# ebiggers/libdeflate

Measured on AMD Instinct MI355X. Metric: compress+decompress MB/s, 64 KiB chunks level 6, higher is better.
Workload: dtype u8

## Files before the change

### libdeflate_amd/csrc/deflate_kernel.hip

```cpp
#include <stddef.h>
#include "device_common.h"
#include "kernels.h"


#ifndef NT
#define NT LDA_DEFLATE_THREADS
#endif
#define VPT (1024 / NT)
#define NWAVES (NT / 64)
#ifndef TILE
#define TILE 4096
#endif
#ifndef RING
#define RING 32768u
#endif
#define RMASK (RING - 1)
#define LOOKAHEAD 272u
#ifndef HASH_BITS
#define HASH_BITS 13
#endif
#ifndef HASH3_BITS
#define HASH3_BITS 12
#endif
#define MAX_BLOCK_LEN 65536u
// ... 507 lines not shown
		const u32 w[4] = { v.x, v.y, v.z, v.w };
#pragma unroll
		for (u32 i = 0; i < 16; i++)
			if (off + i < lim)
				L->seen8[(w[i >> 2] >> (8 * (i & 3))) & 0xFF] = 1;
	}
	wave_sync();
	return wave_sum((u32)__builtin_popcount(s32p[lane] & 0x01010101u));
}

static __device__ __forceinline__ void
stage_input(lds_t *L, const u8 *__restrict__ inp, u32 loaded, u32 want,
	    bool aligned_in, u32 tid)
{
	if (aligned_in) {
		const u32 from = loaded & ~15u;
		for (u32 p = from + tid * 16; p < want; p += NT * 16) {
			uint4 v = *(const uint4 *)(inp + p);
			*(uint4 *)&L->in[p & RMASK] = v;
			if ((p & RMASK) < 32)
				*(uint4 *)&L->in[RING + (p & RMASK)] = v;
		}
	} else {
		for (u32 p = loaded + tid; p < want; p += NT) {
			u8 b = inp[p];
			L->in[p & RMASK] = b;
			if ((p & RMASK) < 32)
				L->in[RING + (p & RMASK)] = b;
		}
	}
}

static __device__ __attribute__((noinline)) void
stage_prefix(lds_t *L, const u8 *__restrict__ pre, u32 n, u32 tid)
{
	stage_input(L, pre, 0, n, true, tid);
}


struct ra_first {
	u32 c16, a0, a1, a2, a3, c3v;
};

static __device__ __forceinline__ struct ra_first
ra_first_loads(const u16 *__restrict__ c3, u32 t, u32 g, u32 lane, bool want3)
{
	struct ra_first f;
	const u32 i = 64 * g + lane, p = t + i;
	const u32 ip = (p & RMASK) & ~3u;

	f.c16 = LDS32(PREV_OFF + ((2 * (p & RMASK)) & ~3u));
	f.a0 = RAW(ip, 0);
	f.a1 = RAW(ip, 4);
	f.a2 = RAW(ip, 8);
	f.a3 = RAW(ip, 12);
	(void)want3;
	f.c3v = *(const u32 *)((const u8 *)c3 + ((2 * (4 + (g < TILE / 64 ? i : lane))) & ~3u));
	return f;
}

template <bool PRE> static __device__ __forceinline__ void
ra_group(lds_t *L, AS3 u32 *Mo, const u16 *__restrict__ c3, u32 t, u32 tend, u32 n,
	 u32 lo_pos, u32 min_len, u32 done_class, u32 nice, u32 dlim3,
	 u32 tag, u32 lane, u32 &g, const struct ra_first &f, struct ra_first &fnext)
{
	const u32 ctr = (u32)offsetof(struct deflate_lds, vars) + 4 * V_CTR;
	const bool want3 = min_len <= 3;
	const u32 i = 64 * g + lane, p = t + i;
	const u32 sp = p & 3;
	const u32 cur = AB(f.a1, f.a0, sp);
	const u64 nxt8 = mk64(AB(f.a2, f.a1, sp), AB(f.a3, f.a2, sp));
	const u32 hsh = 16 * (lane & 1);
	const u32 c3v = want3 ? (f.c3v >> hsh) & 0xFFFF : 0;
	const bool act0 = p < tend && p + 4 <= n;
	const u32 maxlen = n - p < 258 ? n - p : 258;
	const u32 dmaxp = p - lo_pos;
	const u32 nic = nice < maxlen ? nice : maxlen;
	u32 best = 3, bestd = 0;

	const u32 d1 = (p - (f.c16 >> hsh)) & 0xFFFF;
	const bool act1 = act0 && d1 > 0 && d1 <= dmaxp && 3 < nic;
	const u32 cp1 = p - d1;
	const u32 c2 = LDS16(PREV_OFF + 2 * (cp1 & RMASK));
	u32 rn = 0, gn = 0;
	if (PRE)
		rn = claim_issue(ctr);
	const u32 d2 = (p - c2) & 0xFFFF;
	const bool ch2 = act1 && d2 > d1 && d2 <= dmaxp;
	const u32 cp2 = p - d2;
	if (PRE)
		gn = claim_get(rn);
	const u32 c3n = LDS16(PREV_OFF + 2 * (cp2 & RMASK));
	u32 len1, len2;
	match_length2_p(L, act1, ch2, p, cp1, cp2, cur, nxt8, maxlen, lane,
			&len1, &len2, [&]() {
		if (PRE)
			fnext = ra_first_loads(c3, t, gn, lane, want3);
	});
	if (len1 > best) {
		best = len1;
		bestd = d1;
	}
	const bool act2 = ch2 && best < nic;
	if (act2 && len2 > best) {
		best = len2;
		bestd = d2;
	}
	u32 m = best >= 4 && best >= min_len ? best | (bestd << 16) : 0;
	if (m == 0 && want3 && p < tend && p + 3 <= n) {
		u32 b3 = 0;
		u32 bd = find_len3(L, p, cur, c3v, dmaxp, dlim3, &b3);
		if (bd)
			m = 3 | (bd << 16);
	}
	Mo[4 + i] = m;
	const u32 dn = (p - c3n) & 0xFFFF;
	const u32 dcl = act2 && dn > d2 && dn <= dmaxp && best < nic ?
			done_class : DC_FULL;
	L->dhalf[g] = __ballot(dcl >= DC_HALF);
	L->dfull[g] = __ballot(dcl == DC_FULL);
	__builtin_amdgcn_fence(__ATOMIC_RELEASE, "workgroup");
	*(volatile AS3 u32 *)&L->rdy[g] = tag;
	if (PRE) {
		g = gn;
	} else {
		g = claim_get(claim_issue(ctr));
		if (g < TILE / 64)
			fnext = ra_first_loads(c3, t, g, lane, want3);
	}
}

static __device__ __forceinline__ void
round_a_p(lds_t *L, AS3 u32 *Mo, const u16 *__restrict__ c3, u32 t, u32 tend, u32 n,
	  u32 lo_pos, u32 min_len, u32 done_class, u32 nice, u32 dlim3,
	  u32 tag, u32 tid)
{
	const u32 lane = tid & 63;
	const u32 ctr = (u32)offsetof(struct deflate_lds, vars) + 4 * V_CTR;
	u32 g = claim_get(claim_issue(ctr));
	struct ra_first f = { 0, 0, 0, 0, 0, 0 };

	if (g < TILE / 64)
		f = ra_first_loads(c3, t, g, lane, min_len <= 3);
	struct ra_first f2 = { 0, 0, 0, 0, 0, 0 };
#pragma unroll 1
	while (g + RA_PREF_TAIL < TILE / 64) {
		ra_group<true>(L, Mo, c3, t, tend, n, lo_pos, min_len, done_class, nice, dlim3,
			       tag, lane, g, f, f2);
		if (!(g + RA_PREF_TAIL < TILE / 64)) {
			f = f2;
			break;
		}
		ra_group<true>(L, Mo, c3, t, tend, n, lo_pos, min_len, done_class, nice, dlim3,
			       tag, lane, g, f2, f);
	}
#pragma unroll 1
	while (g < TILE / 64)
		ra_group<false>(L, Mo, c3, t, tend, n, lo_pos, min_len, done_class, nice, dlim3,
				tag, lane, g, f, f);
}

static __device__ __forceinline__ void
round_a(lds_t *L, AS3 u32 *Mo, const u16 *__restrict__ c3, u32 t, u32 tend, u32 n,
	u32 lo_pos, u32 min_len, u32 ra_depth, u32 done_class, u32 nice, u32 dlim3,
	u32 tag, u32 tid)
{
	const u32 lane = tid & 63;
	if (ra_depth == 2 && RA_PAIR) {
		round_a_p(L, Mo, c3, t, tend, n, lo_pos, min_len, done_class, nice, dlim3,
			  tag, tid);
		return;
	}

#pragma unroll 1
	for (;;) {
		u32 g = 0;
		if (lane == 0)
			g = atomicAdd((u32 *)&L->vars[V_CTR], 1u);
		g = bcast_first(g);
		if (g >= TILE / 64)
			break;
		const u32 i = 64 * g + lane, p = t + i;
		const u32 c3v = min_len <= 3 ? c3[4 + i] : 0;
		bool act = p < tend && p + 4 <= n;
		const u32 cur = ld32(L->in, p);
		const u64 nxt8 = ld64(L->in, p + 4);
		const u32 maxlen = n - p < 258 ? n - p : 258;
		const u32 dmaxp = p - lo_pos;
		const u32 nic = nice < maxlen ? nice : maxlen;
		u32 c16 = LDS16(PREV_OFF + 2 * (p & RMASK));
		u32 best = 3, bestd = 0, dprev = 0;

		for (u32 s = 0; s < ra_depth; s++) {
			u32 d = (p - c16) & 0xFFFF;
			act = act && d > dprev && d <= dmaxp && best < nic;
			if (!__ballot(act))
				break;
			u32 cp = p - d;
			u32 len = match_length(L, act, p, cp, cur, nxt8, maxlen, lane);
			if (len > best) {
				best = len;
				bestd = d;
			}
			if (act) {
				c16 = LDS16(PREV_OFF + 2 * (cp & RMASK));
				dprev = d;
			}
		}
		u32 m = best >= 4 && best >= min_len ? best | (bestd << 16) : 0;
		if (m == 0 && min_len <= 3 && p < tend && p + 3 <= n) {
			u32 b3 = 0;
			u32 bd = find_len3(L, p, cur, c3v, dmaxp, dlim3, &b3);
			if (bd)
				m = 3 | (bd << 16);
		}
		Mo[4 + i] = m;
		const u32 dn = (p - c16) & 0xFFFF;
		const u32 dcl = act && dn > dprev && dn <= dmaxp && best < nic ?
				done_class : DC_FULL;
		L->dhalf[g] = __ballot(dcl >= DC_HALF);
		L->dfull[g] = __ballot(dcl == DC_FULL);
		__builtin_amdgcn_fence(__ATOMIC_RELEASE, "workgroup");
		*(volatile AS3 u32 *)&L->rdy[g] = tag;
	}
}

static __device__ __forceinline__ void
stage_steps(lds_t *L, s32 limit, u32 mode, u32 nice, u32 tid)
{
	const u32 lane = tid & 63, wave = tid >> 6;

#pragma unroll
	for (u32 k = 0; k < TILE / NT; k++) {
		const u32 g = wave * (TILE / NT) + k, q = 64 * g + lane, idx = q + 4;
		u32 st = 1;
		if ((s32)q < limit)
			st = token_step(L->M[idx], L->M[idx + 1], L->M[idx + 2], mode, nice);
		const u64 b1 = __ballot(st == 1), b2 = __ballot(st == 2);
		if (lane == 0) {
			L->lit1[g] = b1;
			L->lit2[g] = b2;
		}
	}
}

static __device__ __forceinline__ void
stage_steps_claimed(lds_t *L, const AS3 u32 *Ms, s32 limit, u32 mode, u32 nice, u32 tag,
		    u32 lane)
{
	bool had = false;

#pragma unroll 1
	for (;;) {
		if (had)
			lds_add_lane0(VAR_ADDR(V_STDONE), 1u);
		const u32 g = claim_get(claim_issue(VAR_ADDR(V_CTR3)));
		if (g >= TILE / 64)
			break;
		had = true;
		while (*(volatile AS3 u32 *)&L->rdy[g] != tag ||
		       (g + 1 < TILE / 64 && *(volatile AS3 u32 *)&L->rdy[g + 1] != tag))
			__builtin_amdgcn_s_sleep(2);
		__builtin_amdgcn_fence(__ATOMIC_ACQUIRE, "workgroup");
		const u32 q = 64 * g + lane, idx = q + 4;
		u32 st = 1;
		if ((s32)q < limit)
			st = token_step(Ms[idx], Ms[idx + 1], Ms[idx + 2], mode, nice);
		L->lit1A[g] = __ballot(st == 1);
		L->lit2A[g] = __ballot(st == 2);
		__builtin_amdgcn_fence(__ATOMIC_RELEASE, "workgroup");
	}
}

static __device__ __forceinline__ void
stage_steps_cur_claimed(lds_t *L, s32 limit, u32 mode, u32 nice, u32 lane)
{
	bool had = false;

#pragma unroll 1
	for (;;) {
		if (had)
			lds_add_lane0(VAR_ADDR(V_ST2DONE), 1u);
		const u32 g = claim_get(claim_issue(VAR_ADDR(V_CTR4)));
		if (g >= TILE / 64)
			break;
		had = true;
		const u32 q = 64 * g + lane, idx = q + 4;
		u32 st = 1;
		if ((s32)q < limit)
			st = token_step(L->M[idx], L->M[idx + 1], L->M[idx + 2], mode, nice);
		L->lit1[g] = __ballot(st == 1);
		L->lit2[g] = __ballot(st == 2);
		__builtin_amdgcn_fence(__ATOMIC_RELEASE, "workgroup");
	}
}

static __device__ __forceinline__ void wait_lds_eq(lds_t *L, u32 idx, u32 val)
{
	while (*(volatile AS3 u32 *)&L->vars[idx] != val)
		__builtin_amdgcn_s_sleep(2);
	__builtin_amdgcn_fence(__ATOMIC_ACQUIRE, "workgroup");
}

static __device__ __forceinline__ s32
parse_tile(const AS3 u32 *Ms, const AS3 u64 *lit1p, const AS3 u64 *lit2p, AS3 u64 *pmp,
	   u32 lane, s32 entry, s32 limit, u64 *mask_out, u32 max_pass = 0xFFFFFFFFu)
{
	const s32 seg_lo = 64 * (s32)lane;
	const s32 hi = seg_lo + 64 < limit ? seg_lo + 64 : limit;
	const u64 lit = lane < TILE / 64 ? lit1p[lane] : 0;
	const u64 two = lane < TILE / 64 ? lit2p[lane] : 0;
	s32 ein = lane == 0 ? entry : seg_lo;
	s32 q = ein, ex = ein;
	u64 mask = 0, nm = 0;
	bool walking = q < hi;

	{
		const u64 nlit = ~lit;
		const s32 hirel = hi - seg_lo;
		const AS3 u16 *const ml = (const AS3 u16 *)(Ms + 4 + seg_lo);
		u64 starts = 0, ends = 0;
		s32 rel = q - seg_lo;
		while (__ballot(rel < hirel)) {
			if (rel < hirel) {
				const u64 x = nlit >> (u32)rel;
				const u32 left = (u32)(hirel - rel);
				u32 run = (u32)__builtin_ctzll(x | (1ull << 63));
				run = x ? run : 64;
				run = run < left ? run : left;
				const u32 r2 = (u32)rel + run;
				const bool tok = run < left;
				const u32 last = tok ? r2 : r2 - 1;
				starts |= 1ull << (u32)rel;
				ends |= 1ull << last;
				const u32 len = ml[2 * r2];
				const u32 st = (u32)(two >> (r2 & 63)) & 1 ? 2 : len;
				rel = (s32)(tok ? r2 + st : r2);
			}
		}
		if (q < hi) {
			mask = 2 * ends - starts;
			ex = seg_lo + rel;
		}
		walking = false;
	}
	for (;;) {
		while (__ballot(walking)) {
			if (walking) {
				const u32 rel = (u32)(q - seg_lo);
				const u64 inv = ~(lit >> rel);
				u32 run = inv ? (u32)__builtin_ctzll(inv) : 64;
				if (run > (u32)(hi - q))
					run = (u32)(hi - q);
				u64 add = run >= 64 ? ~0ull : (((1ull << run) - 1) << rel);
				q += (s32)run;
				if (q < hi) {
					const u32 r2 = (u32)(q - seg_lo);
					add |= 1ull << r2;
					q += (two >> r2) & 1 ? 2 : (s32)(Ms[4 + q] & 0xFFFF);
				}
				const u64 hit = add & mask;
				if (hit) {
					const u64 below = (hit & (0 - hit)) - 1;
					mask = nm | (add & below) | (mask & ~below);
					walking = false;
				} else {
					nm |= add;
					if (q >= hi) {
						mask = nm;
						ex = q;
						walking = false;
					}
				}
			}
		}
		s32 pe = (s32)__builtin_amdgcn_update_dpp((u32)ex, (u32)ex, 0x138, 0xF, 0xF, false);
		const s32 e = lane == 0 ? entry : pe;
		const bool redo = e != ein && seg_lo < limit;
		if (!__ballot(redo) || --max_pass == 0)
			break;
		nm = 0;
		if (redo) {
			ein = e;
			if (e >= hi) {
				mask = 0;
				ex = e;
			} else {
				q = e;
				walking = true;
			}
		}
	}
	if (lane < TILE / 64)
		pmp[lane] = mask;
	*mask_out = mask;
	return (s32)bcast_lane((u32)ex, limit > 0 ? (u32)(limit - 1) >> 6 : 0);
}

static __device__ __forceinline__ u32
entry_skip(const AS3 u32 *Ms, s32 entry, u32 lim_idx, u32 mode, u32 nice)
{
	u32 e = (u32)(entry + 4);

	for (u32 pre = 0; pre < 2; pre++)
		if (e < 4 && e < lim_idx)
			e += token_step(Ms[e], Ms[e + 1], Ms[e + 2], mode, nice);
	return e;
}

static __device__ __forceinline__ void
parse_and_base(lds_t *L, u32 *__restrict__ tokg, u32 t, s32 limit, u32 mode,
	       u32 nice, u32 lane)
{
	const s32 entry = (s32)bcast_first(L->vars[V_ENTRY]);
	const u32 lim_idx = (u32)(limit + 4);
	const u32 seq0 = bcast_first(L->vars[V_NSEQ]);
	u32 e = (u32)(entry + 4), npre = 0;

	for (u32 pre = 0; pre < 2; pre++) {
		if (e < 4 && e < lim_idx) {
			const u32 mm = L->M[e];
			const u32 st = token_step(mm, L->M[e + 1], L->M[e + 2], mode, nice);
			const u32 l0 = mm & 0xFFFF;
			const bool ism = st == l0 && l0;
			const u32 pos = (u32)((s32)t + (s32)e - 4);
			if (lane == 0) {
				if (ism) {
					u32 sl, xb, xv;
					tokg[seq0 + npre] = TOK_MATCH | (l0 - 3) |
							    (((mm >> 16) - 1) << 8);
					length_code(l0, &sl, &xb, &xv);
					atomicAdd((u32 *)&L->freq[257 + sl], 1u);
					dist_code(mm >> 16, &sl, &xb, &xv);
					atomicAdd((u32 *)&L->freq[288 + sl], 1u);
				} else {
					const u32 b0 = L->in[pos & RMASK];
					tokg[seq0 + npre] = b0;
					atomicAdd((u32 *)&L->freq[b0], 1u);
					if (st == 2) {
						const u32 b1 = L->in[(pos + 1) & RMASK];
						tokg[seq0 + npre + 1] = b1;
						atomicAdd((u32 *)&L->freq[b1], 1u);
					}
				}
			}
			npre += !ism && st == 2 ? 2 : 1;
			e += st;
		}
	}
	u64 mask;
	const s32 px = parse_tile((const AS3 u32 *)L->M, (const AS3 u64 *)L->lit1,
				  (const AS3 u64 *)L->lit2, (AS3 u64 *)L->pm, lane,
				  (s32)e - 4, limit, &mask);
	const u64 two = lane < TILE / 64 ? mask & L->lit2[lane] : 0;
	const u32 cnt = (u32)__builtin_popcountll(mask) + (u32)__builtin_popcountll(two);
	const u32 incl = wave_scan_incl(cnt);
	if (lane < TILE / 64)
		L->gbase[lane] = seq0 + npre + incl - cnt;
	if (lane == 63) {
		L->vars[V_NSEQ] = seq0 + npre + incl;
		L->vars[V_WALKPOS_LO] = (u32)((s32)t + px);
		L->vars[V_ENTRY] = (u32)(px - (s32)TILE);
	}
}

static __device__ __forceinline__ void
emit_groups(lds_t *L, u32 *__restrict__ tokg, u32 t, u32 lane)
{
	const u64 lt = (1ull << lane) - 1;
	bool had = false;

#pragma unroll 1
	for (;;) {
		u32 g = 0;
		asm volatile("s_waitcnt lgkmcnt(0)" ::: "memory");
		if (had)
			lds_add_lane0(VAR_ADDR(V_EMDONE), 1u);
		g = claim_get(claim_issue(VAR_ADDR(V_CTR2)));
		if (g >= TILE / 64)
			break;
		had = true;
		const u64 pmk = L->pm[g];
		if (!pmk)
			continue;
		const u64 two = pmk & L->lit2[g];
		if ((pmk >> lane) & 1) {
			const u32 q = 64 * g + lane, idx = q + 4;
			const u32 m0 = L->M[idx];
			const u32 l0 = m0 & 0xFFFF, dist = m0 >> 16;
			const u32 st = (L->lit1[g] >> lane) & 1 ? 1 : (two >> lane) & 1 ? 2 : l0;
			const u32 o = (t + q) & RMASK;
			const u32 b0 = L->in[o], b1 = L->in[o + 1];
			const u32 lsl = L->lslot[(l0 - 3) & 255];
			const u32 at = L->gbase[g] + (u32)__builtin_popcountll(pmk & lt) +
				       (u32)__builtin_popcountll(two & lt);
			const bool ism = st == l0 && l0;
			u32 dsl, xb, xv;
			dist_code(dist, &dsl, &xb, &xv);
			tokg[at] = ism ? TOK_MATCH | (l0 - 3) | ((dist - 1) << 8) : b0;
			atomicAdd((u32 *)&L->freq[ism ? 257 + lsl : b0], 1u);
			if (ism || st == 2)
				atomicAdd((u32 *)&L->freq[ism ? 288 + dsl : b1], 1u);
			if (!ism && st == 2)
				tokg[at + 1] = b1;
		}
	}
	__builtin_amdgcn_fence(__ATOMIC_RELEASE, "workgroup");
}

static __device__ __forceinline__ u32
build_worklist(lds_t *L, AS3 u32 *W, const AS3 u32 *src, u32 mode, u32 nice, u32 limit, u32 tid)
{
	const u32 lane = tid & 63, wave = tid >> 6;
	const AS3 u32 *Ms = src ? src : (const AS3 u32 *)L->M;

	u64 spill = 0;
	if (mode >= 1 && S3_HALF && wave) {
		const u32 g0 = wave * (TILE / NT), q1 = 64 * g0 - 1;
		const u64 pmask = L->pmA[g0 - 1];
		const u32 l1 = Ms[4 + q1] & 0xFFFF, l2 = Ms[4 + q1 - 1] & 0xFFFF;
		if ((pmask >> 63) && l1 >= 3 && l1 < nice)
			spill = mode >= 2 ? 3 : 1;
		if (mode >= 2 && ((pmask >> 62) & 1) && l2 >= 3 && l2 < nice)
			spill |= 1;
	}
	static_assert(S3_ROUNDS <= 1, "build_worklist() does not record the classes it hands out");
	u32 item[TILE / NT];
	u64 bal[TILE / NT];
	u64 tm_[TILE / NT], dh_[TILE / NT], df_[TILE / NT];
	u32 l0_[TILE / NT];
	u32 cw = 0;
#pragma unroll
	for (u32 k = 0; k < TILE / NT; k++) {
		const u32 g = wave * (TILE / NT) + k, q = 64 * g + lane;
		tm_[k] = L->pmA[g];
		dh_[k] = L->dhalf[g];
		df_[k] = L->dfull[g];
		const u32 mq = Ms[4 + q];
		if (src)
			L->M[4 + q] = mq;
		l0_[k] = mq & 0xFFFF;
	}
#pragma unroll
	for (u32 k = 0; k < TILE / NT; k++) {
		const u32 g = wave * (TILE / NT) + k, q = 64 * g + lane;
		const u64 tmask = bcast64(tm_[k]);
		const bool below = l0_[k] < nice;
		const u64 b = mode >= 1 && S3_HALF ?
			__ballot(lane_bit(tmask) && l0_[k] >= 3 && below) : 0;
		const u64 hmask = (b << 1) | (mode >= 2 ? b << 2 : 0) | spill;
		spill = (b >> 63) | (mode >= 2 ? b >> 62 : 0);
		const u64 wantf = tmask & ~bcast64(df_[k]);
		const u64 wanth = hmask & ~tmask & ~bcast64(dh_[k]);
		const bool isf = lane_bit(wantf);
		bal[k] = __ballot((isf || lane_bit(wanth)) && below);
		item[k] = q | ((isf ? DC_FULL : DC_HALF) << 12);
		cw += (u32)__builtin_popcountll(bal[k]);
	}
	if (lane == 0)
		L->scan[0][wave] = cw;
	__syncthreads();
	const u32 cnt_w = lane < NWAVES ? L->scan[0][lane] : 0;
	const u32 incl_w = wave_scan_incl(cnt_w);
	u32 base = bcast_lane(incl_w - cnt_w, wave);
	const u32 wc = bcast_lane(incl_w, NWAVES - 1);
#pragma unroll
	for (u32 k = 0; k < TILE / NT; k++) {
		const u32 j = base + rank_below(bal[k]);
		if (lane_bit(bal[k]) && j < limit)
			W[j] = item[k];
		base += (u32)__builtin_popcountll(bal[k]);
	}
	if (tid == 0)
		L->qn[0] = 0;
	__syncthreads();
	return bcast_first(wc < limit ? wc : limit);
}

static __device__ __forceinline__ void
search_items(lds_t *L, AS3 u32 *Mo, u32 t, u32 n, u32 lo_pos, u32 min_len, u32 depth,
	     u32 nice, const u16 *W, u32 cnt_items, u32 nwaves, u32 tid)
{
	const u32 lane = tid & 63;
	if ((tid >> 6) >= nwaves)
		return;
	const u32 drain = depth < 8 ? depth : depth >> 3 > 8 ? depth >> 3 : 8;
	const u32 half = depth >> S3_HALF_SHIFT ? depth >> S3_HALF_SHIFT : 1;
	u32 my_i = 0xFFFFFFFFu, p = 0, cur = 0, c16 = 0, dmaxp = 0,
	    maxlen = 0, dep = 0, best = 3, bestd = 0, dprev = 0,
	    cnt = 0, boff = 0, curb = 0, best0 = 3;
	u64 nxt8 = 0, q = 0;
	bool have = false, fin = true, ended = false;
	PROF_SEC_DECL;

	for (;;) {
		PROF_SEC(3);
		u64 mh = __ballot(have);
		u32 nf = __builtin_popcountll(__ballot(fin));
		if (!mh && !nf)
			break;
		if (nf && (nf >= S3_CLAIM || !mh)) {
			const u64 fm = __ballot(fin);
			u32 cbase = 0;
			if (lane == 0)
				cbase = atomicAdd((u32 *)&L->vars[V_CTR], nf);
			cbase = bcast_first(cbase);
			if (fin) {
				if (my_i < TILE && (!W || best > best0))
					Mo[4 + my_i] = best >= 4 && best >= min_len ?
						(best | (bestd << 16)) : 0;
				fin = false;
				my_i = 0xFFFFFFFFu;
				u32 it = cbase + __builtin_popcountll(fm & ((1ull << lane) - 1));
				if (it < cnt_items) {
					u32 item = W ? W[it] : it;
					my_i = item & 0xFFF;
					p = t + my_i;
					if (p + 4 <= n) {
						cur = ld32(L->in, p);
						nxt8 = ld64(L->in, p + 4);
						c16 = LDS16(PREV_OFF + 2 * (p & RMASK));
						maxlen = n - p < 258 ? n - p : 258;
						dmaxp = p - lo_pos;
						best = 3;
						bestd = 0;
						if (W) {
							dep = (item >> 12) == DC_FULL ? depth : half;
							u32 m = Mo[4 + my_i], l0 = m & 0xFFFF;
							if (l0 >= 4) {
								best = l0;
								bestd = m >> 16;
							}
						} else {
							dep = my_i >= TILE - S3_TAIL ? drain : depth;
						}
						best0 = best;
						boff = best - 3;
						curb = boff ? ld32(L->in, p + boff) : cur;
						dprev = 0;
						cnt = 0;
						ended = false;
						have = true;
						if (best >= maxlen) {
							have = false;
							fin = true;
						}
					} else {
						fin = true;
						best = best0 = 3;
					}
				}
			}
			PROF_SEC(0);
			continue;
		}
#pragma unroll
		for (int s = 0; s < S3_WALK; s++) {
			u32 d = (p - c16) & 0xFFFF;
			bool chain = dep && d > dprev && d <= dmaxp;
			bool stall = ended || cnt >= 4;
			bool ok = !stall && chain;
			u32 cp = p - d;
			u32 w = ld32(L->in, cp + boff);
			u32 c16n = LDS16(PREV_OFF + 2 * (cp & RMASK));
			bool hit = ok && w == curb;
			c16 = ok ? c16n : c16;
			dprev = ok ? d : dprev;
			dep -= ok ? 1 : 0;
			ended = ended || (!stall && !chain);
			q = hit ? ((q << 16) | d) : q;
			cnt += hit ? 1 : 0;
		}
		if (!have)
			cnt = 0;
		PROF_SEC(1);
		bool done = false;
		u32 nev = __builtin_popcountll(__ballot(cnt > 0));
		u32 nwalk = __builtin_popcountll(__ballot(have && !ended && cnt < 4));
		while (nev && (nev >= S3_EVMIN || !nwalk)) {
			bool ev = cnt > 0;
			u32 d = (u32)(q >> (16 * ((cnt - 1) & 3))) & 0xFFFF;
			cnt -= ev ? 1 : 0;
			u32 len = match_length(L, ev, p, p - d, cur, nxt8, maxlen, lane);
			if (ev && len > best) {
				best = len;
				bestd = d;
				if (len >= nice || len >= maxlen) {
					done = true;
					cnt = 0;
				} else {
					boff = len - 3;
					curb = ld32(L->in, p + boff);
				}
			}
			if (have && (done || (ended && cnt == 0))) {
				have = false;
				fin = true;
				done = false;
			}
// ... 369 lines not shown
		const bool ra_all = depth <= 4;
		const bool optm = OPT && mode == 3;
		const u32 rounds = optm || ra_all ? 0 : S3_ROUNDS;
		const u32 dlim3 = mode ? 8192u : 4096u;
		const u32 ra_depth = ra_all ? depth : S3_RA_DEPTH;
		const u32 ra_class = ra_all ? DC_FULL :
				     ra_depth >= (depth >> S3_HALF_SHIFT) ? DC_HALF : DC_SHALLOW;
		const u32 wq_limit = mode == 1 && depth < 100 && WQ_LIMIT > 64 * NWAVES ?
				     64 * NWAVES : WQ_LIMIT;
		const bool use3 = level >= 2;
		const bool splits = use3 && n - dict_len >= 5000;
		bool mx_pending = false;
		u32 tail_n = 0, tail_gen = 0, tail_e = 0;
		u32 ml_cur = 3, ml_nxt = 3;
		u32 carryv = 0;

		for (u32 it = 0; it <= num_tiles && !overflow; it++) {
			const bool have_cur = it >= 1;
			const u32 tile = it - 1;
			const u32 t = have_cur ? tile * TILE : 0;
			const u32 tend = t + TILE < n ? t + TILE : n;
			const bool last_tile = it == num_tiles;
			const bool cur_real = have_cur && t >= dict_len;
			const u32 tn = it * TILE;
			const u32 tnend = tn + TILE < n ? tn + TILE : n;
			const bool nxt_real = it < num_tiles && tn >= dict_len;
			const bool have_ins = it + 1 < num_tiles;
			u32 tid_opaque = threadIdx.x;
			asm volatile("" : "+v"(tid_opaque));
			const u32 tid = tid_opaque, lane = tid & 63, wave = tid >> 6;

			PROF_MARK(0);
			if (stored_only) {
				if (!cur_real)
					continue;
				walkpos = tend;
			} else {
				AS3 u32 *const MX = (AS3 u32 *)L->nxtB;
#ifdef LDA_SMALL
				const u32 lo_cur = 0, lo_nxt = 0;
				(void)lo_min;
#else
				const s32 lo_s = (s32)(t + 2 * TILE + LOOKAHEAD) - (s32)RING;
				const u32 lo_cur = lo_s > (s32)lo_min ? (u32)lo_s : lo_min;
				const s32 lo_n = (s32)(tn + 2 * TILE + LOOKAHEAD) - (s32)RING;
				const u32 lo_nxt = lo_n > (s32)lo_min ? (u32)lo_n : lo_min;
#endif
				u16 *c3nxt = c3g + (it & 1) * (TILE + 8);
				u16 *c3ins = c3g + ((it + 1) & 1) * (TILE + 8);
				const s32 limit = last_tile ? (s32)(tend - t) : (s32)TILE - 2;

				const bool wl_copies = cur_real && !optm && rounds && mx_pending;
				if (cur_real) {
					if (mx_pending && !wl_copies)
						for (u32 i = tid; i < TILE; i += NT)
							L->M[4 + i] = MX[4 + i];
					if (tid < 4) {
						L->M[tid] = carryv;
						L->M[TILE + 4 + tid] = 0;
					}
					mx_pending = false;
					ml_cur = ml_nxt;
					for (u32 i = tid; i < 320; i += NT)
						fsave[i] = L->freq[i];
					if (tid == 0) {
						L->vars[V_NSEQ_PRE] = L->vars[V_NSEQ];
						L->vars[V_WPOS_PRE] = walkpos;
					}
					if (!wl_copies)
						__syncthreads();
					PROF_MARK(6);
				}
				const u32 s0_want0 = (it + 2) * TILE + LOOKAHEAD;
				const u32 s0_want = s0_want0 < n ? s0_want0 : n;
				const u32 s0_p = (loaded & ~15u) + tid * 16;
				const bool s0_pre = aligned_in && s0_p < s0_want;
				uint4 s0_v = make_uint4(0, 0, 0, 0);
				if (s0_pre)
					s0_v = *(const uint4 *)(inp + s0_p);
				tail_n = 0;
				if (cur_real && !optm) {
					if (rounds) {
						const u32 wc = build_worklist(L, (AS3 u32 *)L->nxtB,
									      wl_copies ? (const AS3 u32 *)MX : NULL,
									      mode, nice, wq_limit, tid);
						PROF_MARK(39);
						if (wc) {
							AS3 u32 *tl = (AS3 u32 *)L->nxtB;
							search_queue(L, t, n, lo_cur, ml_cur, depth, nice,
								     (AS3 u32 *)L->nxtB, (AS3 u32 *)L->nxtA, wc, tid,
								     nxt_real, &tail_n, &tail_gen, &tl);
							if (tail_n && wave >= 1 && wave <= RB_TAIL_WAVES) {
								const u32 k = 64 * (wave - 1) + lane;
								tail_e = k < tail_n ? tl[k] : 0;
							}
						}
						PROF_MARK(3);
					}
					if (!tail_n)
						stage_steps(L, limit, mode, nice, tid);
				}
				if (cur_real && optm) {
					const bool opt_first = walkpos == block_start;
					const u32 opt_last = level >= 11 ? 2 : 1;
					u32 opt_stage = 0;
					const u32 ent0 = L->vars[V_ENTRY], nseq0 = L->vars[V_NSEQ];
					if (opt_first) {
						for (u32 i = tid; i < TILE + 8; i += NT)
							msave[i] = L->M[i];
						if (tid == 0)
							L->vars[V_FIT] = 0;
					} else {
						const u32 fit = opt_build_costs(L, tid, false, true, t, tend - t, bsave);
						opt_stage = fit ? 0 : 1;
						if (tid == 0) {
							L->vars[V_FIT] = fit;
							if (c == 0) {
								DBG(tile, 6, 100 + fit);
								DBG(tile, 7, L->vars[V_TMP3]);
							}
						}
					}
					for (;;) {
						u32 tid_opaque2 = threadIdx.x;
						asm volatile("" : "+v"(tid_opaque2));
						const u32 tid = tid_opaque2, lane = tid & 63, wave = tid >> 6;
						const u32 s4mode = opt_stage ? 0 : 2;
						if (opt_stage) {
							const s32 ent = (s32)ent0;
							const s32 pend = (s32)(tend - t);
							s32 lo = (s32)(OPT_SEG * wave), hi = lo + OPT_SEG;
							if (wave == 0 && ent < 0)
								lo = ent;
							if (hi > limit)
								hi = limit;
							s32 e = hi + OPT_WARM;
							if (e > pend)
								e = pend;
							if (lo < hi)
								opt_parse_wave(L, L->nxtA, t, lo, hi, e, lane);
							__syncthreads();
							for (s32 i = (s32)tid + (ent < 0 ? ent : 0); i < limit; i += NT) {
								u32 c = L->nxtA[i + 4], m = L->M[i + 4];
								L->M[i + 4] = c >= 3 ? c | (m & 0xFFFF0000u) : 0;
							}
							__syncthreads();
						}
						stage_steps(L, limit, s4mode, nice, tid);
						if (tid == 0)
							L->vars[V_CTR2] = 0;
						__syncthreads();
						if (wave == 0)
							parse_and_base(L, tokg, t, limit, s4mode, nice, lane);
						__syncthreads();
						PROF_MARK(12);
						emit_groups(L, tokg, t, lane);
						__syncthreads();
						PROF_MARK(5);
						if (!opt_first || opt_stage == opt_last)
							break;
						opt_build_costs(L, tid, opt_stage == 0, false, t, tend - t, bsave);
						for (u32 i = tid; i < 320; i += NT)
							L->freq[i] = 0;
						for (u32 i = tid; i < TILE + 8; i += NT)
							L->M[i] = msave[i];
						if (tid == 0) {
							L->vars[V_ENTRY] = ent0;
							L->vars[V_NSEQ] = nseq0;
						}
						__syncthreads();
						opt_stage++;
					}
				}

				{
					const u32 want = s0_want;
					if (s0_pre) {
						*(uint4 *)&L->in[s0_p & RMASK] = s0_v;
						if ((s0_p & RMASK) < 32)
							*(uint4 *)&L->in[RING + (s0_p & RMASK)] = s0_v;
					}
					if (aligned_in) {
						if ((loaded & ~15u) + NT * 16 < want)
							stage_input(L, inp, (loaded & ~15u) + NT * 16, want, true, tid);
					} else {
						stage_input(L, inp, loaded, want, false, tid);
					}
					loaded = want > loaded ? want : loaded;
					if (tid == 0) {
						L->vars[V_CTR] = 0;
						L->vars[V_CTR2] = 0;
						L->vars[V_CTR3] = 0;
						L->vars[V_STDONE] = 0;
						L->vars[V_EMDONE] = 0;
						L->vars[V_TAILDONE] = 0;
						L->vars[V_CTR4] = 0;
						L->vars[V_ST2DONE] = 0;
					}
					if (tid < 4 && nxt_real) {
						AS3 u32 *const Mo = cur_real ? MX : (AS3 u32 *)L->M;
						if (!tail_n)
							Mo[tid] = cur_real ? L->M[TILE + tid] : 0;
						Mo[TILE + 4 + tid] = 0;
					}
					if (nxt_real && it)
						ml_nxt = bcast_first(L->vars[V_MINLEN]);
					__syncthreads();
				}
				PROF_MARK(1);
				if (it == 0) {
					if (wave == NWAVES - 1)
						insert_tile(L, 0, tnend, n, lane);
					if (wave == NWAVES - 2 && use3) {
						insert_tile3(L, c3nxt, 0, tnend, n, lane);
						__builtin_amdgcn_fence(__ATOMIC_RELEASE, "workgroup");
					}
					if (wave == NWAVES - 3 && nxt_real) {
						const u32 nd = wave_distinct_bytes(L, 0, loaded < TILE ? loaded : TILE, lane);
						if (lane == 0)
							L->vars[V_MINLEN] = min_len_policy(nd, n - dict_len, depth, use3);
					}
					__syncthreads();
					if (nxt_real)
						ml_nxt = bcast_first(L->vars[V_MINLEN]);
					PROF_MARK(2);
				}
				__builtin_amdgcn_fence(__ATOMIC_ACQUIRE, "workgroup");

				{
					const bool do_p2 = cur_real && !optm;
					AS3 u32 *const Mo = cur_real ? MX : (AS3 u32 *)L->M;
					PROF_WDECL;
					PROF_W0();
					if (wave == NWAVES - 1) {
						__builtin_amdgcn_s_setprio(3);
						if (have_ins)
							insert_tile(L, tnend, tnend + TILE < n ? tnend + TILE : n,
								    n, lane);
						__builtin_amdgcn_s_setprio(0);
						PROF_W(24);
					} else if (wave == NWAVES - 2) {
						__builtin_amdgcn_s_setprio(2);
						if (have_ins && use3) {
							insert_tile3(L, c3ins, tnend,
								     tnend + TILE < n ? tnend + TILE : n, n, lane);
							__builtin_amdgcn_fence(__ATOMIC_RELEASE, "workgroup");
						}
						__builtin_amdgcn_s_setprio(0);
						if (have_ins && tnend >= dict_len) {
							const u32 nd = wave_distinct_bytes(L, tnend,
								loaded - tnend < TILE ? loaded - tnend : TILE, lane);
							if (lane == 0)
								L->vars[V_MINLEN] = min_len_policy(nd, n - dict_len, depth, use3);
						}
						PROF_W(25);
					} else if (wave == 0 && do_p2) {
						if (tail_n)
							wait_lds_eq(L, V_ST2DONE, TILE / 64);
						__builtin_amdgcn_s_setprio(3);
						parse_and_base(L, tokg, t, limit, mode, nice, lane);
						__builtin_amdgcn_fence(__ATOMIC_RELEASE, "workgroup");
						if (lane == 0)
							*(volatile AS3 u32 *)&L->vars[V_PFLAG] = it;
						__builtin_amdgcn_s_setprio(0);
						if (tail_n && nxt_real && lane < 4)
							Mo[lane] = L->M[TILE + lane];
						PROF_W(26);
					} else if (RB_DEFER && tail_n && wave <= RB_TAIL_WAVES) {
						__builtin_amdgcn_s_setprio(2);
						if (64 * (wave - 1) < tail_n) {
							u32 nx;
							(void)rb_batch(L, t, n, lo_nxt, ml_cur, rb_trim_depth(depth), nice,
								       tail_e, tail_e != 0, tail_gen, lane, &nx);
						}
						__builtin_amdgcn_fence(__ATOMIC_RELEASE, "workgroup");
						if (lane == 0)
							atomicAdd((u32 *)&L->vars[V_TAILDONE], 1u);
						wait_lds_eq(L, V_TAILDONE, RB_TAIL_WAVES);
						stage_steps_cur_claimed(L, limit, mode, nice, lane);
						__builtin_amdgcn_s_setprio(0);
					}
					if (nxt_real) {
						if (optm) {
							if (wave < NWAVES - 2)
								search_items(L, Mo, tn, n, lo_nxt, ml_nxt, depth, nice,
									     NULL, TILE, NWAVES - 2, tid);
						} else {
							round_a(L, Mo, c3nxt, tn, tnend, n, lo_nxt, ml_nxt, ra_depth,
								ra_class, nice, dlim3, it + 1, tid);
						}
					}
					if (wave == 1)
						PROF_W(27);
					if (nxt_real && rounds) {
						const s32 lim_n = it + 1 == num_tiles ? (s32)(tnend - tn) : (s32)TILE - 2;
						stage_steps_claimed(L, Mo, lim_n, mode, nice, it + 1, lane);
						if (wave == 0) {
							u64 mk;
							wait_lds_eq(L, V_STDONE, TILE / 64);
							const u32 e = entry_skip(Mo, (s32)L->vars[V_ENTRY],
										 (u32)(lim_n + 4), mode, nice);
							(void)parse_tile(Mo, (const AS3 u64 *)L->lit1A,
									 (const AS3 u64 *)L->lit2A, (AS3 u64 *)L->pmA,
									 lane, (s32)e - 4, lim_n, &mk, P1_PASSES);
						}
						if (wave == 1)
							PROF_W(33);
						if (wave == 0)
							PROF_W(34);
					}
					if (do_p2) {
						while (*(volatile AS3 u32 *)&L->vars[V_PFLAG] != it)
							__builtin_amdgcn_s_sleep(4);
						__builtin_amdgcn_fence(__ATOMIC_ACQUIRE, "workgroup");
						if (wave == 1)
							PROF_W(28);
						emit_groups(L, tokg, t, lane);
						if (wave == 1)
							PROF_W(29);
						if (wave == NWAVES - 1 && splits && !last_tile) {
							wait_lds_eq(L, V_EMDONE, TILE / 64);
							split_stats(L, bcast_first(L->vars[V_WALKPOS_LO]), block_start, false, lane);
						}
					}
					__syncthreads();
					if (wave == 1)
						PROF_W(30);
					if (wave == 0)
						PROF_W(31);
					if (optm && nxt_real) {
						PROF_MARK(16);
						if (ml_nxt <= 3) {
							for (u32 i = tid; i < TILE; i += NT) {
								u32 p = tn + i, b3 = 0;
								if (p + 3 <= n && Mo[4 + i] == 0) {
									u32 bd = find_len3(L, p, ld32(L->in, p),
											   c3nxt[4 + i], p - lo_nxt,
											   dlim3, &b3);
									if (bd)
										Mo[4 + i] = 3 | (bd << 16);
								}
							}
						}
						__syncthreads();
					}
					mx_pending = cur_real && nxt_real;
				}
				PROF_MARK(4);
				if (!cur_real)
					continue;

				if (OPT && mode == 3)
					walkpos = bcast_first(L->vars[V_WALKPOS_LO]);
				if (tid < 4)
					carryv = L->M[TILE + tid];
				if (splits && wave == NWAVES - 1 && optm) {
					split_stats(L, walkpos, block_start, L->vars[V_FIT] == 2, lane);
				}
			}
			if (OPT && mode == 3)
				__syncthreads();
			PROF_MARK(32);

			u32 splitv, nseq_now;
			if (OPT && mode == 3) {
				splitv = splits && !stored_only && !last_tile ?
					 bcast_first(L->vars[V_SPLIT]) : 0;
				nseq_now = stored_only ? 0 : bcast_first(L->vars[V_NSEQ]);
			} else {
				const uint4 pv = *(const AS3 uint4 *)&L->vars[V_NSEQ];
				static_assert(V_NSEQ == 0 && V_WALKPOS_LO == 2 && V_SPLIT == 3, "one 16-byte read");
				if (!stored_only)
					walkpos = bcast_first(pv.z);
				splitv = splits && !stored_only && !last_tile ? bcast_first(pv.w) : 0;
				nseq_now = stored_only ? 0 : bcast_first(pv.x);
			}
			bool end_block = last_tile || splitv ||
				(!stored_only && nseq_now - blk_tok0 + 2 * TOK_TILE_MAX > TOK_CAP) ||
				walkpos - block_start > MAX_BLOCK_LEN;
			if (!end_block)
				continue;
			if (tid < 10)
				L->obs[0][tid] = 0;

			const bool retro = splitv == 2;
			const u32 bstart = block_start;
			const u32 bend = last_tile ? n : retro ? bcast_first(L->vars[V_WPOS_PRE]) : walkpos;
			const u32 blen = bend - bstart;
			const u32 nseq_all = nseq_now;
			const u32 nseq = retro ? bcast_first(L->vars[V_NSEQ_PRE]) : nseq_all;
			const u32 is_final = last_tile && seg_last ? 1 : 0;
			if (SPLIT) {
				u32 *d = blk_desc + (size_t)nblocks * LDA_BLK_WORDS;
				for (u32 i = tid; i < 320; i += NT) {
					const u32 f = L->freq[i], fp = retro ? fsave[i] : f;
					d[LDA_BLK_FREQ + i] = fp;
					L->freq[i] = f - fp;
				}
				if (tid == 0) {
					d[LDA_BLK_TOK0] = blk_tok0;
					d[LDA_BLK_NTOK] = nseq - blk_tok0;
					d[LDA_BLK_START] = bstart;
					d[LDA_BLK_END] = bend;
					d[LDA_BLK_FLAGS] = is_final | (stored_only ? LDA_BLK_STORED : 0);
				}
				nblocks++;
				blk_tok0 = nseq;
				carryv = 0;
				block_start = bend;
				__syncthreads();
				continue;
			}
			if (retro) {
				for (u32 i = tid; i < 320; i += NT) {
					u32 f = L->freq[i], fp = fsave[i];
					fsave[320 + i] = f - fp;
					L->freq[i] = fp;
				}
				__syncthreads();
			}

			if (!stored_only && mx_pending) {
				const AS3 u32 *MXs = (const AS3 u32 *)L->nxtB;
				for (u32 i = tid; i < TILE; i += NT)
					msave[4 + i] = MXs[4 + i];
			}
			PROF_MARK(10);
			if (!block_emit(L, &os, tokg, nseq, inp, bstart, blen, is_final, stored_only,
					ftr_bytes, &tog, tid, lane, wave)) {
				overflow = true;
				break;
			}
			PROF_START();
			if (OPT && mode == 3 && tid < 256)
				bsave[tid] = 0;
			if (retro) {
				const u32 cnt = nseq_all - nseq;
				enum { RPT = (TOK_TILE_MAX + NT - 1) / NT };
				u32 mv[RPT];
#pragma unroll
				for (u32 k = 0; k < RPT; k++)
					mv[k] = tid + NT * k < cnt ? tokg[nseq + tid + NT * k] : 0;
				__syncthreads();
#pragma unroll
				for (u32 k = 0; k < RPT; k++)
					if (tid + NT * k < cnt)
						tokg[tid + NT * k] = mv[k];
				for (u32 i = tid; i < 320; i += NT)
					L->freq[i] = fsave[320 + i];
				if (tid == 0)
					L->vars[V_NSEQ] = cnt;
				__builtin_amdgcn_fence(__ATOMIC_RELEASE, "workgroup");
			} else {
				for (u32 i = tid; i < 320; i += NT)
					L->freq[i] = 0;
				if (tid == 0)
					L->vars[V_NSEQ] = 0;
			}
			carryv = 0;
			if (mx_pending) {
				for (u32 i = tid; i < TILE; i += NT)
					L->M[4 + i] = msave[4 + i];
				mx_pending = false;
			}
			block_start = bend;
			__syncthreads();
		}

		if (SPLIT) {
			__syncthreads();
			if (tid == 0) {
				blk_buf[c] = over_bound ? LDA_BLK_FUSED :
					     overflow ? LDA_BLK_OVERFLOW : nblocks;
				if (over_bound)
					blk_buf[LDA_BLK_LIST(n_chunks) + atomicAdd(fused_cnt, 1u)] = (u32)c;
			}
		} else {
			finish_stream(L, &os, overflow, seg_last, format, ftr_bytes, sums, c, n,
				      out_nbytes, tid);
		}
	}
}

#define DEFLATE_KERNEL_PARAMS                                                  \
	u64 n_chunks, int format, int level, u32 depth, u32 nice, u32 mode,    \
	const u8 *__restrict__ in_base, const u64 *__restrict__ in_offsets,    \
	const u64 *__restrict__ in_nbytes, u8 *__restrict__ out_base,          \
	const u64 *__restrict__ out_offsets,                                   \
	const u64 *__restrict__ out_avail_arr, u64 *__restrict__ out_nbytes,   \
	const u32 *__restrict__ sums, u64 *__restrict__ seq_scratch,           \
	const u32 *__restrict__ seg_info, u32 *__restrict__ next_chunk,       \
	const u8 *__restrict__ dict_pre
#define DEFLATE_KERNEL_ARGS                                                    \
	lds_raw, n_chunks, format, level, depth, nice, mode, in_base,          \
	in_offsets, in_nbytes, out_base, out_offsets, out_avail_arr,           \
	out_nbytes, sums, seq_scratch, seg_info, next_chunk, dict_pre

#ifdef LDA_SMALL
extern "C" __global__ void __launch_bounds__(NT, SMALL_WGS)
lda_deflate_small_kernel(DEFLATE_KERNEL_PARAMS)
{
	extern __shared__ __attribute__((aligned(16))) u8 lds_raw[];
	deflate_batch_body<false>(DEFLATE_KERNEL_ARGS);
}

extern "C" size_t lda_deflate_small_lds_bytes(void)
{
	return sizeof(struct deflate_lds);
}

extern "C" size_t lda_deflate_small_max(void)
{
	return RING;
}

extern "C" size_t lda_deflate_small_wgs(void)
{
	return SMALL_WGS;
}

LDA_PROF_DEFINE_READER(libdeflate_amd_profile_read_deflate_small)
#else
extern "C" __global__ void __launch_bounds__(NT)
lda_deflate_batch_kernel(DEFLATE_KERNEL_PARAMS, u32 *__restrict__ tok_buf,
			 u32 *__restrict__ blk_buf, u32 tok_stride, u32 blk_stride,
			 u32 *__restrict__ fused_cnt)
{
	extern __shared__ __attribute__((aligned(16))) u8 lds_raw[];
	deflate_batch_body<false, true>(DEFLATE_KERNEL_ARGS, tok_buf, blk_buf, tok_stride,
					blk_stride, fused_cnt);
}

extern "C" __global__ void __launch_bounds__(NT)
lda_deflate_fused_kernel(DEFLATE_KERNEL_PARAMS, const u32 *__restrict__ blk_buf,
			 const u32 *__restrict__ fused_cnt)
{
	extern __shared__ __attribute__((aligned(16))) u8 lds_raw[];
	deflate_batch_body<false>(DEFLATE_KERNEL_ARGS, NULL, (u32 *)blk_buf, 0, 0,
				  (u32 *)fused_cnt);
}

extern "C" __global__ void __launch_bounds__(NT)
lda_deflate_opt_kernel(DEFLATE_KERNEL_PARAMS)
{
	extern __shared__ __attribute__((aligned(16))) u8 lds_raw[];
	deflate_batch_body<true>(DEFLATE_KERNEL_ARGS);
}

extern "C" size_t lda_deflate_lds_bytes(void)
{
	return sizeof(struct deflate_lds);
}

extern "C" size_t lda_deflate_tile(void)
{
	return TILE;
}

extern "C" size_t lda_deflate_seq_words(void)
{
	return SEQ_STRIDE;
}

LDA_PROF_DEFINE_READER(libdeflate_amd_profile_read_deflate)

#endif
```

Measured before the change: 34520.

## Split per-lane 64-position parse walk into two independent 32-bit halves

Rewrites the wave-parallel token parse so that each lane walks two 32-position halves of its 64-position segment side by side, using 32-bit masks and branch-free step updates. The intent is to shorten the serial dependency chain per lane and use cheaper 32-bit bit operations, with a speculative seed walk followed by fix-up passes that now also chain from half A into half B. Optional profiling counters are added behind LDA_PROFILE. In exchange, each lane does more work per step and the redo logic becomes more complex, which could add iterations.

```diff
diff --git a/libdeflate_amd/csrc/deflate_kernel.hip b/libdeflate_amd/csrc/deflate_kernel.hip
--- a/libdeflate_amd/csrc/deflate_kernel.hip
+++ b/libdeflate_amd/csrc/deflate_kernel.hip
@@ -833,99 +833,170 @@
 	__builtin_amdgcn_fence(__ATOMIC_ACQUIRE, "workgroup");
 }
 
+#ifdef LDA_PROFILE
+#define PW_DECL u32 pw_it1_ = 0, pw_np_ = 0, pw_it2_ = 0; \
+	const unsigned long long pw_t0_ = __builtin_readcyclecounter()
+#define PW_IT1() (pw_it1_++)
+#define PW_PASS() (pw_np_++)
+#define PW_IT2() (pw_it2_++)
+#define PW_FLUSH(slot) do { if (lane == 0) { \
+	atomicAdd(&lda_prof[slot], __builtin_readcyclecounter() - pw_t0_); \
+	atomicAdd(&lda_prof[43], (unsigned long long)pw_it1_); \
+	atomicAdd(&lda_prof[44], (unsigned long long)pw_np_); \
+	atomicAdd(&lda_prof[45], (unsigned long long)pw_it2_); \
+	atomicAdd(&lda_prof[46], 1ull); \
+	atomicMax(&lda_prof[47], (unsigned long long)pw_it1_); } } while (0)
+#else
+#define PW_DECL
+#define PW_IT1() do { } while (0)
+#define PW_PASS() do { } while (0)
+#define PW_IT2() do { } while (0)
+#define PW_FLUSH(slot) do { } while (0)
+#endif
+
+struct walk_half {
+	s32 base;
+	s32 hr;
+	u32 lit, two;
+	u32 valid;
+	s32 ein, ex;
+	s32 rel;
+	u32 mask, nm;
+};
+
+static __device__ __forceinline__ u32
+walk_stretch(const walk_half &h, s32 rel)
+{
+	const u32 y = ~h.lit & (~0u << ((u32)rel & 31));
+	const u32 r2 = y ? (u32)__builtin_ctz(y) : 32;
+
+	return r2 < (u32)h.hr ? r2 : (u32)h.hr;
+}
+
+static __device__ __forceinline__ s32
+walk_land(const walk_half &h, u32 r2, bool tok, u32 len)
+{
+	const u32 st = (h.two >> (r2 & 31)) & 1 ? 2 : len;
+
+	return (s32)(r2 + (tok ? st : 0));
+}
+
+static __device__ __forceinline__ void
+walk2_step(walk_half &h, u32 r2, u32 len)
+{
+	const bool w = h.rel < h.hr;
+	const bool tok = r2 < (u32)h.hr;
+	const s32 nr = walk_land(h, r2, tok, len);
+	const u32 str = ((h.lit + (1u << ((u32)h.rel & 31))) ^ h.lit) & h.valid;
+	const u32 hit = str & h.mask;
+	const u32 below = (hit & (0 - hit)) - 1;
+	const u32 path = h.nm | (str & below) | (h.mask & ~below);
+	const bool out = nr >= h.hr;
+	const bool fin = hit != 0 || out;
+
+	h.mask = w && fin ? path : h.mask;
+	h.nm = w && !fin ? path : h.nm;
+	h.ex = w && !hit && out ? h.base + nr : h.ex;
+	h.rel = w ? (hit ? 32 : nr) : h.rel;
+}
+
+static __device__ __forceinline__ void
+walk_redo(walk_half &h, s32 e, bool redo)
+{
+	h.nm = 0;
+	if (redo) {
+		h.ein = e;
+		if (e >= h.base + h.hr) {
+			h.mask = 0;
+			h.ex = e;
+		} else {
+			h.rel = e - h.base;
+		}
+	}
+}
+
 static __device__ __forceinline__ s32
 parse_tile(const AS3 u32 *Ms, const AS3 u64 *lit1p, const AS3 u64 *lit2p, AS3 u64 *pmp,
-	   u32 lane, s32 entry, s32 limit, u64 *mask_out, u32 max_pass = 0xFFFFFFFFu)
-{
+	   u32 lane, s32 entry, s32 limit, u64 *mask_out, u32 max_pass = 0xFFFFFFFFu,
+	   u32 prof_slot = 41)
+{
+	PW_DECL;
 	const s32 seg_lo = 64 * (s32)lane;
-	const s32 hi = seg_lo + 64 < limit ? seg_lo + 64 : limit;
 	const u64 lit = lane < TILE / 64 ? lit1p[lane] : 0;
 	const u64 two = lane < TILE / 64 ? lit2p[lane] : 0;
-	s32 ein = lane == 0 ? entry : seg_lo;
-	s32 q = ein, ex = ein;
-	u64 mask = 0, nm = 0;
-	bool walking = q < hi;
+	walk_half A, B;
+
+	A.base = seg_lo;
+	B.base = seg_lo + 32;
+	A.hr = limit - A.base < 0 ? 0 : limit - A.base < 32 ? limit - A.base : 32;
+	B.hr = limit - B.base < 0 ? 0 : limit - B.base < 32 ? limit - B.base : 32;
+	A.valid = A.hr >= 32 ? ~0u : (1u << A.hr) - 1;
+	B.valid = B.hr >= 32 ? ~0u : (1u << B.hr) - 1;
+	A.lit = (u32)lit;
+	B.lit = (u32)(lit >> 32);
+	A.two = (u32)two;
+	B.two = (u32)(two >> 32);
+	A.ein = lane == 0 ? entry : A.base;
+	B.ein = B.base;
+	A.ex = A.ein;
+	B.ex = B.ein;
+	A.rel = A.ein - A.base;
+	B.rel = 0;
+	A.mask = A.nm = B.mask = B.nm = 0;
+	const AS3 u16 *const mlA = (const AS3 u16 *)(Ms + 4 + (lane < TILE / 64 ? seg_lo : 0));
+	const AS3 u16 *const mlB = mlA + 64;
 
 	{
-		const u64 nlit = ~lit;
-		const s32 hirel = hi - seg_lo;
-		const AS3 u16 *const ml = (const AS3 u16 *)(Ms + 4 + seg_lo);
-		u64 starts = 0, ends = 0;
-		s32 rel = q - seg_lo;
-		while (__ballot(rel < hirel)) {
-			if (rel < hirel) {
-				const u64 x = nlit >> (u32)rel;
-				const u32 left = (u32)(hirel - rel);
-				u32 run = (u32)__builtin_ctzll(x | (1ull << 63));
-				run = x ? run : 64;
-				run = run < left ? run : left;
-				const u32 r2 = (u32)rel + run;
-				const bool tok = run < left;
-				const u32 last = tok ? r2 : r2 - 1;
-				starts |= 1ull << (u32)rel;
-				ends |= 1ull << last;
-				const u32 len = ml[2 * r2];
-				const u32 st = (u32)(two >> (r2 & 63)) & 1 ? 2 : len;
-				rel = (s32)(tok ? r2 + st : r2);
-			}
-		}
-		if (q < hi) {
-			mask = 2 * ends - starts;
-			ex = seg_lo + rel;
-		}
-		walking = false;
-	}
+		const bool hadA = A.rel < A.hr, hadB = B.rel < B.hr;
+		u32 landA = 0, landB = 0;
+
+		if (__ballot((A.rel < A.hr) | (B.rel < B.hr))) do {
+			const bool actA = A.rel < A.hr, actB = B.rel < B.hr;
+			PW_IT1();
+			const u32 rA = walk_stretch(A, A.rel), rB = walk_stretch(B, B.rel);
+			const u32 lenA = mlA[2 * rA], lenB = mlB[2 * rB];
+			landA |= (u32)actA << ((u32)A.rel & 31);
+			landB |= (u32)actB << ((u32)B.rel & 31);
+			const s32 nA = walk_land(A, rA, actA && rA < (u32)A.hr, lenA);
+			const s32 nB = walk_land(B, rB, actB && rB < (u32)B.hr, lenB);
+			A.rel = A.rel > nA ? A.rel : nA;
+			B.rel = B.rel > nB ? B.rel : nB;
+		} while (__ballot((A.rel < A.hr) | (B.rel < B.hr)));
+		if (hadA) {
+			A.mask = ((A.lit + landA) ^ A.lit) & A.valid;
+			A.ex = A.base + A.rel;
+		}
+		if (hadB) {
+			B.mask = ((B.lit + landB) ^ B.lit) & B.valid;
+			B.ex = B.base + B.rel;
+		}
+	}
+	s32 exl;
 	for (;;) {
-		while (__ballot(walking)) {
-			if (walking) {
-				const u32 rel = (u32)(q - seg_lo);
-				const u64 inv = ~(lit >> rel);
-				u32 run = inv ? (u32)__builtin_ctzll(inv) : 64;
-				if (run > (u32)(hi - q))
-					run = (u32)(hi - q);
-				u64 add = run >= 64 ? ~0ull : (((1ull << run) - 1) << rel);
-				q += (s32)run;
-				if (q < hi) {
-					const u32 r2 = (u32)(q - seg_lo);
-					add |= 1ull << r2;
-					q += (two >> r2) & 1 ? 2 : (s32)(Ms[4 + q] & 0xFFFF);
-				}
-				const u64 hit = add & mask;
-				if (hit) {
-					const u64 below = (hit & (0 - hit)) - 1;
-					mask = nm | (add & below) | (mask & ~below);
-					walking = false;
-				} else {
-					nm |= add;
-					if (q >= hi) {
-						mask = nm;
-						ex = q;
-						walking = false;
-					}
-				}
-			}
-		}
-		s32 pe = (s32)__builtin_amdgcn_update_dpp((u32)ex, (u32)ex, 0x138, 0xF, 0xF, false);
-		const s32 e = lane == 0 ? entry : pe;
-		const bool redo = e != ein && seg_lo < limit;
-		if (!__ballot(redo) || --max_pass == 0)
+		if (__ballot((A.rel < A.hr) | (B.rel < B.hr))) do {
+			PW_IT2();
+			const u32 rA = walk_stretch(A, A.rel), rB = walk_stretch(B, B.rel);
+			const u32 lenA = mlA[2 * rA], lenB = mlB[2 * rB];
+			walk2_step(A, rA, lenA);
+			walk2_step(B, rB, lenB);
+		} while (__ballot((A.rel < A.hr) | (B.rel < B.hr)));
+		exl = B.base < limit ? B.ex : A.ex;
+		const s32 pe = (s32)__builtin_amdgcn_update_dpp((u32)exl, (u32)exl, 0x138, 0xF, 0xF, false);
+		const s32 enA = lane == 0 ? entry : pe, enB = A.ex;
+		const bool redoA = enA != A.ein && A.base < limit;
+		const bool redoB = enB != B.ein && B.base < limit;
+		if (!__ballot(redoA | redoB) || --max_pass == 0)
 			break;
-		nm = 0;
-		if (redo) {
-			ein = e;
-			if (e >= hi) {
-				mask = 0;
-				ex = e;
-			} else {
-				q = e;
-				walking = true;
-			}
-		}
-	}
+		PW_PASS();
+		walk_redo(A, enA, redoA);
+		walk_redo(B, enB, redoB);
+	}
+	const u64 mask = A.mask | (u64)B.mask << 32;
 	if (lane < TILE / 64)
 		pmp[lane] = mask;
 	*mask_out = mask;
-	return (s32)bcast_lane((u32)ex, limit > 0 ? (u32)(limit - 1) >> 6 : 0);
+	PW_FLUSH(prof_slot);
+	return (s32)bcast_lane((u32)exl, limit > 0 ? (u32)(limit - 1) >> 6 : 0);
 }
 
 static __device__ __forceinline__ u32
@@ -1901,7 +1972,7 @@
 										 (u32)(lim_n + 4), mode, nice);
 							(void)parse_tile(Mo, (const AS3 u64 *)L->lit1A,
 									 (const AS3 u64 *)L->lit2A, (AS3 u64 *)L->pmA,
-									 lane, (s32)e - 4, lim_n, &mk, P1_PASSES);
+									 lane, (s32)e - 4, lim_n, &mk, P1_PASSES, 42);
 						}
 						if (wave == 1)
 							PROF_W(33);
```

Result: no change. 34660, median of 6 (+0.4%).
